# ericehanley/gke-ray-train

Hardware: AMD Instinct MI355X
Metric: tokens/sec (whole node) Llama-2-7B fine-tune at 1/2/4/8 MI355X; samples/sec on Wikitext-2 (higher is better)
Workload: dtype bf16; 1 GPU; model=llama2-7b, global_batch=8, seq_len=1024, parallelism=dp1, micro_batch=8, grad_accum=1, optimizer=fused AdamW fp32 states, activation_checkpointing=False, optimizer_overlap=True, forced_collectives=False, library_gemms=offline-tuned

## Files before the change

gke_ray_train_amd/csrc/bindings/ops.cpp:

```cpp
#include <climits>
#include <torch/extension.h>

#include <algorithm>
#include <cmath>
#include <c10/hip/HIPStream.h>
#include <c10/core/DeviceGuard.h>

#include "grt_kernels.h"
#include "grt_sdma.h"

namespace {

using at::Tensor;
using c10::optional;

hipStream_t cur_stream(const Tensor& t) {
  return c10::hip::getCurrentHIPStream(t.device().index()).stream();
}

grt::DType dtype_of(const Tensor& t) {
  if (t.scalar_type() == at::kBFloat16) return grt::DType::BF16;
  TORCH_CHECK(t.scalar_type() == at::kFloat, "gke_ray_train_amd kernels support bf16/fp32, got ", t.scalar_type());
  return grt::DType::F32;
}
// ... 697 lines not shown
  if (p.drop_thresh == 0) p.drop_thresh = 1;
  p.drop_scale = (float)(1.0 / (1.0 - dropout_p));
}

std::vector<Tensor> attn_fwd(const Tensor& q, const Tensor& k, const Tensor& v, const optional<Tensor>& out,
                             double scale, bool causal, const optional<Tensor>& seqlens_k, double dropout_p,
                             int64_t seed, const optional<Tensor>& cu_seqlens, int64_t max_seqlen,
                             const optional<Tensor>& o_t) {
  c10::OptionalDeviceGuard g(q.device());
  Tensor o = out.has_value() ? *out : at::empty(q.sizes(), q.options());
  auto lse = cu_seqlens.has_value()
                 ? at::empty({cu_seqlens->numel() - 1, q.size(2), max_seqlen}, q.options().dtype(at::kFloat))
                 : at::empty({q.size(0), q.size(2), q.size(1)}, q.options().dtype(at::kFloat));
  auto p = make_params(q, k, v, o, lse, scale, causal, seqlens_k, cu_seqlens, max_seqlen);
  set_dropout(p, dropout_p, seed);
  if (o_t.has_value()) {
    check_contig(*o_t, "o_t");
    TORCH_CHECK(q.scalar_type() == at::kBFloat16 && p.D == 128 && o_t->scalar_type() == at::kBFloat16 &&
                    o_t->dim() == 2 && o_t->size(0) == (int64_t)p.Hq * p.D && o_t->size(1) == q.size(0) * q.size(1),
                "attn_fwd o_t: bf16, head_dim 128, shape [Hq * D, B * S]");
    p.o_t = o_t->data_ptr();
    p.ot_ld = o_t->size(1);
  }
  if (q.scalar_type() == at::kFloat) grt::attn_fwd_f32(p, cur_stream(q));
  else grt::attn_fwd(p, cur_stream(q));
  return {o, lse};
}

std::vector<Tensor> attn_bwd(const Tensor& dout, const Tensor& q, const Tensor& k, const Tensor& v, const Tensor& o,
                             Tensor& lse, const optional<Tensor>& dq_out, const optional<Tensor>& dk_out,
                             const optional<Tensor>& dv_out, double scale, bool causal,
                             const optional<Tensor>& seqlens_k, double dropout_p, int64_t seed,
                             const optional<Tensor>& rope_cos, const optional<Tensor>& rope_sin,
                             const optional<Tensor>& cu_seqlens, int64_t max_seqlen, const optional<Tensor>& dqkv_t) {
  c10::OptionalDeviceGuard g(q.device());
  check_bshd(dout, "dout");
  TORCH_CHECK(dout.sizes() == q.sizes(), "dout shape");
  auto p = make_params(q, k, v, o, lse, scale, causal, seqlens_k, cu_seqlens, max_seqlen);
  set_dropout(p, dropout_p, seed);
  Tensor dq = dq_out.has_value() ? *dq_out : at::empty(q.sizes(), q.options());
  Tensor dk = dk_out.has_value() ? *dk_out : at::empty(k.sizes(), k.options());
  Tensor dv = dv_out.has_value() ? *dv_out : at::empty(v.sizes(), v.options());
  check_bshd(dq, "dq");
  check_bshd(dk, "dk");
  check_bshd(dv, "dv");
  TORCH_CHECK(dq.sizes() == q.sizes() && dk.sizes() == k.sizes() && dv.sizes() == v.sizes(), "grad shapes");
  auto ws = at::empty({grt::attn_bwd_workspace_floats(p.B, p.Hq, p.Sq, p.D)}, q.options().dtype(at::kFloat));
  grt::AttnBwdParams bp{};
  bp.f = p;
  bp.dout = dout.data_ptr(); bp.do_bs = dout.stride(0); bp.do_ss = dout.stride(1); bp.do_hs = dout.stride(2);
  bp.dq = dq.data_ptr(); bp.dq_bs = dq.stride(0); bp.dq_ss = dq.stride(1); bp.dq_hs = dq.stride(2);
  bp.dk = dk.data_ptr(); bp.dk_bs = dk.stride(0); bp.dk_ss = dk.stride(1); bp.dk_hs = dk.stride(2);
  bp.dv = dv.data_ptr(); bp.dv_bs = dv.stride(0); bp.dv_ss = dv.stride(1); bp.dv_hs = dv.stride(2);
  if (cu_seqlens.has_value()) bp.do_bs = bp.dq_bs = bp.dk_bs = bp.dv_bs = 0;
  bp.delta = ws.data_ptr<float>();
  TORCH_CHECK(rope_cos.has_value() == rope_sin.has_value(), "attn_bwd: rope_cos and rope_sin together");
  if (rope_cos.has_value()) {
    check_contig(*rope_cos, "rope_cos");
    check_contig(*rope_sin, "rope_sin");
    TORCH_CHECK(q.scalar_type() == at::kBFloat16 && p.D == 128, "attn_bwd rope epilogue: bf16, head_dim 128");
    TORCH_CHECK(rope_cos->scalar_type() == at::kFloat && rope_sin->sizes() == rope_cos->sizes() &&
                    rope_sin->scalar_type() == at::kFloat && rope_cos->dim() == 2 && rope_cos->size(1) == p.D / 2 &&
                    rope_cos->size(0) >= std::max(p.Sq, p.Sk),
                "attn_bwd: rope tables fp32 [>= max(Sq, Sk), D / 2]");
    bp.rope_cos = rope_cos->data_ptr<float>();
    bp.rope_sin = rope_sin->data_ptr<float>();
  }
  TORCH_CHECK(dout.scalar_type() == q.scalar_type() && dq.scalar_type() == q.scalar_type() &&
                  dk.scalar_type() == q.scalar_type() && dv.scalar_type() == q.scalar_type(), "grad dtype mismatch");
  if (dqkv_t.has_value()) {
    check_contig(*dqkv_t, "dqkv_t");
    TORCH_CHECK(q.scalar_type() == at::kBFloat16 && p.D == 128 && dqkv_t->scalar_type() == at::kBFloat16,
                "attn_bwd dqkv_t: bf16, head_dim 128");
    TORCH_CHECK(p.Sq == p.Sk && dqkv_t->dim() == 2 && dqkv_t->size(0) == (int64_t)(p.Hq + 2 * p.Hkv) * p.D &&
                    dqkv_t->size(1) == q.size(0) * q.size(1),
                "attn_bwd dqkv_t: self-attention, shape [(Hq + 2 Hkv) * D, B * S]");
    bp.dqkv_t = dqkv_t->data_ptr();
    bp.t_ld = dqkv_t->size(1);
    bp.t_row_q = 0;
    bp.t_row_k = p.Hq * p.D;
    bp.t_row_v = (p.Hq + p.Hkv) * p.D;
  }
  if (q.scalar_type() == at::kFloat) grt::attn_bwd_f32(bp, cur_stream(q));
  else grt::attn_bwd(bp, cur_stream(q));
  return {dq, dk, dv};
}

Tensor attn_decode(const Tensor& q, const Tensor& k, const Tensor& v, const optional<Tensor>& seqlens_k, double scale) {
  check_bshd(q, "q");
  check_bshd(k, "k");
  check_bshd(v, "v");
  TORCH_CHECK(q.scalar_type() == at::kBFloat16 && k.scalar_type() == at::kBFloat16 && v.scalar_type() == at::kBFloat16,
              "attn_decode: bf16");
  TORCH_CHECK(q.size(1) == 1, "attn_decode: one query token per sequence");
  TORCH_CHECK(k.sizes() == v.sizes() && k.size(0) == q.size(0), "attn_decode: k/v shapes");
  const int64_t Hq = q.size(2), Hkv = k.size(2);
  TORCH_CHECK(Hq % Hkv == 0, "attn_decode: Hq % Hkv");
  const int64_t G = Hq / Hkv;
  TORCH_CHECK(G == 1 || G == 2 || G == 4 || G == 8, "attn_decode: GQA group must be 1, 2, 4 or 8");
  c10::OptionalDeviceGuard g(q.device());
  grt::AttnDecodeParams p{};
  p.q = q.data_ptr(); p.k = k.data_ptr(); p.v = v.data_ptr();
  auto o = at::empty(q.sizes(), q.options());
  p.o = o.data_ptr();
  p.q_bs = q.stride(0); p.q_hs = q.stride(2);
  p.k_bs = k.stride(0); p.k_ss = k.stride(1); p.k_hs = k.stride(2);
  p.v_bs = v.stride(0); p.v_ss = v.stride(1); p.v_hs = v.stride(2);
  p.o_bs = o.stride(0); p.o_hs = o.stride(2);
  p.B = (int)q.size(0); p.Hq = (int)Hq; p.Hkv = (int)Hkv; p.Sk = (int)k.size(1);
  p.NS = grt::attn_decode_splits(p.B, p.Hkv, p.Sk);
  p.seqlens_k = nullptr;
  if (seqlens_k.has_value()) {
    check_contig(*seqlens_k, "seqlens_k");
    TORCH_CHECK(seqlens_k->scalar_type() == at::kInt && seqlens_k->numel() == q.size(0), "seqlens_k int32 [B]");
    p.seqlens_k = seqlens_k->data_ptr<int32_t>();
  }
  p.scale_log2 = (float)(scale * 1.4426950408889634);
// ... 436 lines not shown
        py::arg("want_xd"), py::arg("h_out") = py::none(), py::arg("hscale") = 1.0);
  m.def("lora_dx", &lora_dx, py::arg("g"), py::arg("at"), py::arg("dx"), py::arg("p"), py::arg("seed"),
        py::arg("offset"), py::arg("accumulate"), py::arg("dx_in") = py::none(), py::arg("gscale") = 1.0);
  m.def("lora_refresh", &lora_refresh, py::arg("bs"), py::arg("offs"), py::arg("w"), py::arg("wt"), py::arg("col0"),
        py::arg("wt_row0") = -1);
  m.def("lora_g", &lora_g, py::arg("a"), py::arg("bt"), py::arg("c"), py::arg("alpha"), py::arg("accumulate"));
  m.def("lora_g_group", &lora_g_group, py::arg("a"), py::arg("bt"), py::arg("c"), py::arg("alpha"),
        py::arg("accumulate"));
  m.def("lora_tred", &lora_tred, py::arg("a"), py::arg("h"), py::arg("out"), py::arg("alpha"), py::arg("accumulate"),
        py::arg("transpose"));
  m.def("lora_tred_group", &lora_tred_group, py::arg("a"), py::arg("h"), py::arg("out"), py::arg("alpha"),
        py::arg("accumulate"));
  m.def("dropout_bwd_seeded", &dropout_bwd_seeded);
  m.def("ce_fwd", &ce_fwd);
  m.def("ce_bwd", &ce_bwd);
  m.def("sumsq_blocks", &sumsq_blocks);
  m.def("lds_fill", [](int64_t pattern, int64_t device) {
    c10::OptionalDeviceGuard g(c10::Device(c10::DeviceType::CUDA, (c10::DeviceIndex)device));
    grt::lds_fill((uint32_t)pattern, c10::hip::getCurrentHIPStream((c10::DeviceIndex)device).stream());
  }, "test support: fill every CU's LDS with a 32-bit pattern (stale-LDS-read detection)");
  m.def("sumsq", &sumsq);
  m.def("clip_finalize", &clip_finalize);
  m.def("adamw", &adamw, py::arg("p"), py::arg("g"), py::arg("m"), py::arg("v"), py::arg("master"),
        py::arg("hyper"), py::arg("gscale"), py::arg("max_blocks") = 0, py::arg("index_offset") = 0);
  m.def("adamw_t", &adamw_t);
  m.def("scale_", &scale_);
  m.def("attn_fwd", &attn_fwd, py::arg("q"), py::arg("k"), py::arg("v"), py::arg("out"), py::arg("scale"),
        py::arg("causal"), py::arg("seqlens_k"), py::arg("dropout_p") = 0.0, py::arg("seed") = 0,
        py::arg("cu_seqlens") = py::none(), py::arg("max_seqlen") = 0, py::arg("o_t") = py::none());
  m.def("attn_bwd", &attn_bwd, py::arg("dout"), py::arg("q"), py::arg("k"), py::arg("v"), py::arg("o"),
        py::arg("lse"), py::arg("dq"), py::arg("dk"), py::arg("dv"), py::arg("scale"), py::arg("causal"),
        py::arg("seqlens_k"), py::arg("dropout_p") = 0.0, py::arg("seed") = 0, py::arg("rope_cos") = py::none(),
        py::arg("rope_sin") = py::none(), py::arg("cu_seqlens") = py::none(), py::arg("max_seqlen") = 0,
        py::arg("dqkv_t") = py::none());
  m.def("attn_set_schedule", &grt::attn_set_schedule,
        "bf16 attention causal-pair / XCD-grouped schedule, bit mask: 1 = forward, 2 = dQ, 4 = dK/dV");
  m.def("attn_get_schedule", &grt::attn_get_schedule);
  m.def("attn_set_dkdv_form", &grt::attn_set_dkdv_form, "dK / dV kernel: 1 = 4-wave, 2 = wave-pair (default)");
  m.def("attn_get_dkdv_form", &grt::attn_get_dkdv_form);
  m.def("attn_set_dma_fast", &grt::attn_set_dma_fast, "1 = hoisted LDS-DMA addressing (default), 0 = clamped per tile");
  m.def("ew_set_fast", &grt::ew_set_fast, "1 = single-pass RoPE (D = 128) / SwiGLU kernels (default), 0 = grid-stride kernels");
  m.def("attn_set_skip_dead", &grt::attn_set_skip_dead,
        "1 = forward / dK-dV waves skip the causal tiles they mask entirely (default), 0 = compute them");
  m.def("nf4_quantize", &nf4_quantize);
  m.def("nf4_dequantize", &nf4_dequantize);
  m.def("nf4_dequantize_t", &nf4_dequantize_t);
  m.def("nf4_dequantize_into", &nf4_dequantize_into);
  m.def("rmsnorm_bwd_dx", &rmsnorm_bwd_dx);
  m.def("swiglu_fwd_t", &swiglu_fwd_t);
  m.def("swiglu_bwd_t", &swiglu_bwd_t);
  m.def("transpose_into", &transpose_into);
  m.def("copy_sdma", &copy_sdma);
  m.def("sdma_d2h", &sdma_d2h, py::arg("dst"), py::arg("src"), py::arg("producer_stream") = 0,
        "pinned host <- device on an SDMA engine, ordered on the source's current stream; producer_stream "
        "(a raw stream handle): the stream whose work so far wrote src");
  m.def("sdma_stats", &sdma_stats, "copies / bytes / worker busy seconds / first error of the SDMA copier");
  m.def("sdma_clear_error", [](int64_t device) { grt::sdma_clear_error((int)device); });
  m.def("gemv", &gemv, py::arg("x"), py::arg("w"), py::arg("swiglu") = false);
  m.def("gemv_fused", &gemv_fused, py::arg("x"), py::arg("w"), py::arg("sumsq"), py::arg("slot"),
        py::arg("swiglu") = false, py::arg("g") = py::none(), py::arg("res") = py::none(), py::arg("eps") = 1e-5,
        py::arg("cos") = py::none(), py::arg("sin") = py::none(), py::arg("pos") = py::none(),
        py::arg("kc") = py::none(), py::arg("vc") = py::none(), py::arg("hq") = 0, py::arg("hkv") = 0);
  m.def("attn_decode", &attn_decode);
  m.def("embedding_fwd", &embedding_fwd);
  m.def("embedding_bwd", &embedding_bwd);
  m.def("gemm_wgrad", &gemm_wgrad, py::arg("x"), py::arg("y"), py::arg("out"), py::arg("accumulate"),
        py::arg("mode") = 0);
// ... 18 lines not shown
```

gke_ray_train_amd/csrc/kernels/attention.hip:

```cpp
#include <limits.h>
#include <stdlib.h>

#include <type_traits>
#include <utility>

#include "grt_common.h"
#include "grt_kernels.h"

namespace grt {
namespace {

typedef __attribute__((address_space(3))) bf16x4 lds_bf16x4;

constexpr int D = 128;
constexpr int kChunks = D / 8;

__device__ __forceinline__ f32x16 mfma32(bf16x8 a, bf16x8 b, f32x16 c) {
  return __builtin_amdgcn_mfma_f32_32x32x16_bf16(a, b, c, 0, 0, 0);
}

__device__ __forceinline__ int img_off(int row, int ch) {
  return row * 256 + 16 * (ch ^ (((row & 3) << 2) | ((row >> 2) & 3)));
}
__device__ __forceinline__ bf16x8 lds_row_read(const char* base, int row, int ch) {
// ... 6 lines not shown
  return __builtin_amdgcn_ds_read_tr16_b64_v4bf16((lds_bf16x4*)a);
}

__device__ __forceinline__ bf16x8 cat(bf16x4 a, bf16x4 b) {
  return __builtin_shufflevector(a, b, 0, 1, 2, 3, 4, 5, 6, 7);
}
__device__ __forceinline__ bf16x8 pack8(const f32x16& x, int base) {
  bf16x8 r;
#pragma unroll
  for (int j = 0; j < 8; ++j) r[j] = static_cast<bf16>(x[base + j]);
  return r;
}
__device__ __forceinline__ int acc_row(int r, int h) { return (r & 3) + 8 * (r >> 2) + 4 * h; }

__device__ __forceinline__ uint32_t fmix32(uint32_t h) {
  h ^= h >> 16; h *= 0x85ebca6bu; h ^= h >> 13; h *= 0xc2b2ae35u; h ^= h >> 16;
  return h;
}
__device__ __forceinline__ uint32_t attn_dropout_hash(uint32_t seed, uint32_t bh, uint32_t q, uint32_t k) {
  uint32_t h = seed ^ (bh * 0x9E3779B1u);
  h = fmix32(h ^ (q * 0x85EBCA77u));
  return fmix32(h ^ (k * 0xC2B2AE3Du));
}
__device__ __forceinline__ float drop_factor(const AttnParams& p, uint32_t bh, int q, int k) {
  return attn_dropout_hash(p.drop_seed, bh, (uint32_t)q, (uint32_t)k) >= p.drop_thresh ? p.drop_scale : 0.f;
}

constexpr float kLog2e = 1.4426950408889634f;
constexpr float kLn2 = 0.6931471805599453f;

__device__ __forceinline__ float halves_max(float x) {
  const auto r = __builtin_amdgcn_permlane32_swap(__float_as_uint(x), __float_as_uint(x), false, false);
  return fmaxf(__uint_as_float(r[0]), __uint_as_float(r[1]));
}

constexpr float kDeferLog2 = 8.f;

__device__ __forceinline__ void lds_dma16(const void* gptr, uint32_t lds_byte_addr) {
  asm volatile("s_mov_b32 m0, %1\n\ts_nop 0\n\tglobal_load_lds_dwordx4 %0, off"
               :: "v"(gptr), "s"(lds_byte_addr) : "memory", "m0");
}
__device__ __forceinline__ uint32_t lds_u32(const void* p) {
  return (uint32_t)(uintptr_t)(const __attribute__((address_space(3))) char*)(p);
}
__device__ __forceinline__ int img_swz(int row) { return ((row & 3) << 2) | ((row >> 2) & 3); }

template <class F, int... I>
__device__ __forceinline__ void static_for(F&& f, std::integer_sequence<int, I...>) {
  (f(std::integral_constant<int, I>{}), ...);
}
__device__ __forceinline__ void wait_tiles4(int tiles) {
  if (tiles >= 4) asm volatile("s_waitcnt vmcnt(16)" ::: "memory");
  else if (tiles == 3) asm volatile("s_waitcnt vmcnt(12)" ::: "memory");
  else if (tiles == 2) asm volatile("s_waitcnt vmcnt(8)" ::: "memory");
  else if (tiles == 1) asm volatile("s_waitcnt vmcnt(4)" ::: "memory");
  else asm volatile("s_waitcnt vmcnt(0)" ::: "memory");
}

constexpr int F3M = 128, F3N = 32, F3NT = 256, F3NSLOT = 4;
constexpr int F3IMG = F3N * D * 2;
constexpr int F3SLOT = 2 * F3IMG;

struct QJobs {
  int bh;
  int blk0, blk1;
};
// ... 212 lines not shown
        a.v[j] = static_cast<bf16>(o[db][8 * gp + j] * inv);
        c2.v[j] = static_cast<bf16>(o[db][8 * gp + 4 + j] * inv);
      }
      const auto r0 = __builtin_amdgcn_permlane32_swap(a.u[0], c2.u[0], false, false);
      const auto r1 = __builtin_amdgcn_permlane32_swap(a.u[1], c2.u[1], false, false);
      if (myq < Sq) {
        *reinterpret_cast<uint4*>(O + db * 32 + 16 * gp + 8 * h) = make_uint4(r0[0], r1[0], r0[1], r1[1]);
        if (p.o_t != nullptr) {
          bf16* ot = static_cast<bf16*>(p.o_t) + (int64_t)(hq * D) * p.ot_ld + (p.cu_seqlens ? 0 : (int64_t)b * p.Sq) +
                     tok0 + myq;
          const int d0 = db * 32 + 8 * (2 * gp) + 4 * h, d1 = db * 32 + 8 * (2 * gp + 1) + 4 * h;
#pragma unroll
          for (int j = 0; j < 4; ++j) {
            ot[(int64_t)(d0 + j) * p.ot_ld] = a.v[j];
            ot[(int64_t)(d1 + j) * p.ot_ld] = c2.v[j];
          }
        }
      }
    }
  if (myq < Sq) {
    if (h == 0 && p.lse)
      p.lse[((int64_t)b * p.Hq + hq) * p.Sq + myq] = lt > 0.f ? (m + __log2f(lt)) * kLn2 : INFINITY;
  }
  };
  run_block(jobs.blk0);
  if (jobs.blk1 >= 0) {
    asm volatile("s_waitcnt lgkmcnt(0)" ::: "memory");
    __builtin_amdgcn_s_barrier();
    run_block(jobs.blk1);
  }
}

__host__ __device__ inline int sq_pad(int Sq) { return (Sq + 31) / 32 * 32; }

__global__ __launch_bounds__(256) void attn_bwd_pre_kernel(const AttnBwdParams p) {
  const int l16 = threadIdx.x & 15;
  const int Sqp = sq_pad(p.f.Sq);
  const int64_t row = (int64_t)blockIdx.x * 16 + (threadIdx.x >> 4);
  const int64_t nrows = (int64_t)p.f.B * p.f.Hq * Sqp;
  if (row >= nrows) return;
  const int q = (int)(row % Sqp);
  const int64_t bh = row / Sqp;
  float acc = 0.f;
  const int hq = (int)(bh % p.f.Hq), b = (int)(bh / p.f.Hq);
  int Sq = p.f.Sq;
  int64_t tok0 = 0;
  if (p.f.cu_seqlens) {
    tok0 = p.f.cu_seqlens[b];
    Sq = p.f.cu_seqlens[b + 1] - (int)tok0;
  }
  if (q < Sq) {
    const bf16* O = (const bf16*)p.f.o + (int64_t)b * p.f.o_bs + (int64_t)hq * p.f.o_hs + (tok0 + q) * p.f.o_ss;
    const bf16* dO = (const bf16*)p.dout + (int64_t)b * p.do_bs + (int64_t)hq * p.do_hs + (tok0 + q) * p.do_ss;
    float a[8], g[8];
    load16(O + l16 * 8, a);
    load16(dO + l16 * 8, g);
#pragma unroll
    for (int k = 0; k < 8; ++k) acc += a[k] * g[k];
  }
#pragma unroll
  for (int o = 8; o >= 1; o >>= 1) acc += __shfl_xor(acc, o, 16);
  if (l16 == 0) {
    float* lse2 = p.delta + nrows;
    p.delta[row] = acc;
    lse2[row] = q < Sq ? p.f.lse[bh * p.f.Sq + q] * kLog2e : INFINITY;
  }
}


struct TCopy {
  bf16* p;
  int64_t ld;
};
__device__ __forceinline__ void st_t(const TCopy& tc, int d, const bf16x4& v) {
  if (tc.p != nullptr) {
#pragma unroll
    for (int j = 0; j < 4; ++j) tc.p[(int64_t)(d + j) * tc.ld] = v[j];
  }
}
__device__ __forceinline__ TCopy tcopy(const AttnBwdParams& P, int row0, int head, int64_t tok) {
  if (P.dqkv_t == nullptr) return TCopy{nullptr, 0};
  return TCopy{static_cast<bf16*>(P.dqkv_t) + (int64_t)(row0 + head * D) * P.t_ld + tok, P.t_ld};
}

__device__ __forceinline__ void store_unrotated(const f32x16 (&acc)[4], float scale, const float* __restrict__ cr,
                                                const float* __restrict__ sr, bf16* dst, int h,
                                                const TCopy& tc = TCopy{nullptr, 0}) {
#pragma unroll
  for (int db = 0; db < 2; ++db)
#pragma unroll
    for (int gg = 0; gg < 4; ++gg) {
      const int d = db * 32 + 8 * gg + 4 * h;
      const f32x4 c = *reinterpret_cast<const f32x4*>(cr + d);
      const f32x4 sn = *reinterpret_cast<const f32x4*>(sr + d);
      bf16x4 lo, hi;
#pragma unroll
      for (int j = 0; j < 4; ++j) {
        const float x1 = acc[db][4 * gg + j] * scale, x2 = acc[db + 2][4 * gg + j] * scale;
        lo[j] = static_cast<bf16>(x1 * c[j] + x2 * sn[j]);
        hi[j] = static_cast<bf16>(x2 * c[j] - x1 * sn[j]);
      }
// ... 536 lines not shown
  auto run_role = [&](auto role_c) __attribute__((always_inline)) {
    run_block(jobs.blk0, role_c);
    if (jobs.blk1 >= 0) {
      asm volatile("s_waitcnt lgkmcnt(0)" ::: "memory");
      __builtin_amdgcn_s_barrier();
      run_block(jobs.blk1, role_c);
    }
  };
  if (swave) run_role(std::true_type{});
  else run_role(std::false_type{});
}

constexpr int Q2M = 128, Q2N = 32, Q2NT = 256, Q2NSLOT = 4;
constexpr int Q2IMG = Q2N * D * 2;
constexpr int Q2SLOT = 2 * Q2IMG;

template <bool DROP>
__global__ __launch_bounds__(Q2NT, 2) void attn_bwd_dq_kernel(const AttnBwdParams P) {
  const AttnParams& p = P.f;
  __shared__ __attribute__((aligned(16))) char smem[Q2NSLOT * Q2SLOT];
  const int tid = threadIdx.x, lane = tid & 63, h = lane >> 5, l32 = lane & 31;
  const int w = __builtin_amdgcn_readfirstlane(tid >> 6);
  const int g = lane >> 4, l16 = lane & 15;
  const int nqb = (p.Sq + Q2M - 1) / Q2M;
  const int BH = p.B * p.Hq;
  const QJobs jobs = q_jobs(p.sched, nqb, BH);
  const int bh = jobs.bh;
  const int b = bh / p.Hq, hq = bh % p.Hq;
  const int hkv = hq / (p.Hq / p.Hkv);
  GRT_DEVICE_CHECK(b < p.B && hkv < p.Hkv && jobs.blk0 >= 0 && jobs.blk0 < nqb);
  auto run_block = [&](const int qblk) {
  int Sq = p.Sq, Sk = p.Sk;
  int64_t tok0 = 0;
  if (p.cu_seqlens) {
    tok0 = p.cu_seqlens[b];
    Sq = Sk = p.cu_seqlens[b + 1] - (int)tok0;
    if (qblk * Q2M >= Sq) return;
  }
  const int sk = p.seqlens_k ? min(Sk, p.seqlens_k[b]) : Sk;
  const int off = Sk - Sq;
  const int q0 = qblk * Q2M, qw0 = q0 + w * 32;
  const int myq = qw0 + l32;
  const bool qok = myq < Sq;
  const int Sqp = sq_pad(p.Sq);

  const bf16* Q = (const bf16*)p.q + (int64_t)b * p.q_bs + tok0 * p.q_ss + (int64_t)hq * p.q_hs;
  const bf16* dO = (const bf16*)P.dout + (int64_t)b * P.do_bs + tok0 * P.do_ss + (int64_t)hq * P.do_hs;
  const bf16* K = (const bf16*)p.k + (int64_t)b * p.k_bs + tok0 * p.k_ss + (int64_t)hkv * p.k_hs;
  const bf16* Vg = (const bf16*)p.v + (int64_t)b * p.v_bs + tok0 * p.v_ss + (int64_t)hkv * p.v_hs;

  bf16x8 qf[D / 16], of[D / 16];
#pragma unroll
  for (int ks = 0; ks < D / 16; ++ks) {
    if (qok) {
      qf[ks] = *reinterpret_cast<const bf16x8*>(Q + (int64_t)myq * p.q_ss + ks * 16 + 8 * h);
      of[ks] = *reinterpret_cast<const bf16x8*>(dO + (int64_t)myq * P.do_ss + ks * 16 + 8 * h);
    } else {
      qf[ks] = bf16x8{};
      of[ks] = bf16x8{};
    }
  }
  const int64_t ri = (int64_t)bh * Sqp + min(myq, Sqp - 1);
  const float lse2 = P.delta[(int64_t)BH * Sqp + ri];
  const float dlt = P.delta[ri];
  const float c = p.scale * kLog2e;
  const int klim = p.causal ? min(sk - 1, myq + off) : sk - 1;
  const int kmask = p.causal ? min(sk, qw0 + off + 1) : sk;
  const int klast = p.skip_dead && p.causal && !DROP ? min(sk - 1, qw0 + 31 + off) : INT_MAX;

  int kend = sk;
  if (p.causal) kend = min(kend, q0 + Q2M + off);
  const int nt = kend > 0 ? (kend + Q2N - 1) / Q2N : 0;

  const uint32_t smem0 = lds_u32(smem);
  const int row0 = 8 * w + g, row1 = row0 + 4;
  const int ch0 = l16 ^ img_swz(row0), ch1 = l16 ^ img_swz(row1);
  auto dma_tile = [&](int t, uint32_t slot_off) {
    const int64_t k0r = min(t * Q2N + row0, Sk - 1), k1r = min(t * Q2N + row1, Sk - 1);
    const uint32_t dst = __builtin_amdgcn_readfirstlane(smem0 + slot_off + (uint32_t)(8 * w * 256));
    lds_dma16(K + k0r * p.k_ss + ch0 * 8, dst);
    lds_dma16(Vg + k0r * p.v_ss + ch0 * 8, dst + Q2IMG);
    lds_dma16(K + k1r * p.k_ss + ch1 * 8, dst + 1024);
    lds_dma16(Vg + k1r * p.v_ss + ch1 * 8, dst + Q2IMG + 1024);
  };
  auto wait_dma = [&](int pending_tiles) {
    if (pending_tiles >= 2) asm volatile("s_waitcnt vmcnt(8)" ::: "memory");
    else if (pending_tiles == 1) asm volatile("s_waitcnt vmcnt(4)" ::: "memory");
    else asm volatile("s_waitcnt vmcnt(0)" ::: "memory");
  };
  auto sdp = [&](int t, auto slot_c, f32x16& s, f32x16& dp) {
    constexpr int SL = decltype(slot_c)::value;
    const char* ki = smem + SL * Q2SLOT;
    const int kb = t * Q2N;
    s = f32x16{};
    if (kb + Q2N > kmask) {
#pragma unroll
      for (int r = 0; r < 16; ++r) s[r] = kb + acc_row(r, h) <= klim ? 0.f : -INFINITY;
// ... 24 lines not shown
  for (int i = 0; i < 4; ++i) dq[i] = f32x16{};

  using I0 = std::integral_constant<int, 0>;
  auto step = [&](int t, auto slot_c, f32x16& s_c, f32x16& dp_c, f32x16& s_n, f32x16& dp_n) {
    constexpr int SL = decltype(slot_c)::value;
    asm volatile("s_waitcnt lgkmcnt(0)" ::: "memory");
    if (t + 1 < nt) wait_dma(min(nt, t + Q2NSLOT - 1) - (t + 2));
    __builtin_amdgcn_s_barrier();
    if (t + Q2NSLOT - 1 < nt) dma_tile(t + Q2NSLOT - 1, (uint32_t)(((SL + Q2NSLOT - 1) % Q2NSLOT) * Q2SLOT));
    if (t * Q2N > klast) return;

    sdp(t + 1, std::integral_constant<int, (SL + 1) % Q2NSLOT>{}, s_n, dp_n);

#pragma unroll
    for (int r = 0; r < 16; ++r) {
      const float pv = fast_exp2(fmaf(s_c[r], c, -lse2));
      const float z = DROP ? drop_factor(p, (uint32_t)bh, myq, t * Q2N + acc_row(r, h)) : 1.f;
      s_c[r] = pv * (dp_c[r] * z - dlt);
    }
    const char* ki = smem + SL * Q2SLOT;
#pragma unroll
    for (int stp = 0; stp < 2; ++stp) {
      const bf16x8 sb = pack8(s_c, 8 * stp);
      const int kk = 16 * stp + 4 * h;
#pragma unroll
      for (int db = 0; db < 4; ++db) {
        const int c0 = db * 32 + (g & 1) * 16;
        const bf16x8 a = cat(lds_tr_read(ki, kk, c0, l16), lds_tr_read(ki, kk + 8, c0, l16));
        dq[db] = mfma32(a, sb, dq[db]);
      }
    }
  };

  if (nt > 0) {
    const int pre = min(nt, Q2NSLOT - 1);
    for (int t = 0; t < pre; ++t) dma_tile(t, (uint32_t)(t * Q2SLOT));
    wait_dma(pre - 1);
    __builtin_amdgcn_s_barrier();
    f32x16 sA, dpA, sB, dpB;
    sdp(0, I0{}, sA, dpA);
    int t = 0;
    for (; t + Q2NSLOT <= nt; t += Q2NSLOT) {
      step(t, I0{}, sA, dpA, sB, dpB);
      step(t + 1, std::integral_constant<int, 1>{}, sB, dpB, sA, dpA);
      step(t + 2, std::integral_constant<int, 2>{}, sA, dpA, sB, dpB);
      step(t + 3, std::integral_constant<int, 3>{}, sB, dpB, sA, dpA);
    }
    if (t < nt) step(t, I0{}, sA, dpA, sB, dpB);
    if (t + 1 < nt) step(t + 1, std::integral_constant<int, 1>{}, sB, dpB, sA, dpA);
    if (t + 2 < nt) step(t + 2, std::integral_constant<int, 2>{}, sA, dpA, sB, dpB);
  }
  asm volatile("s_waitcnt vmcnt(0)" ::: "memory");

  if (qok) {
    bf16* dQ = (bf16*)P.dq + (int64_t)b * P.dq_bs + (int64_t)hq * P.dq_hs + (tok0 + myq) * P.dq_ss;
    const TCopy tq = tcopy(P, P.t_row_q, hq, (p.cu_seqlens ? 0 : (int64_t)b * p.Sq) + tok0 + myq);
    if (P.rope_cos) {
      store_unrotated(dq, p.scale, P.rope_cos + (int64_t)myq * (D / 2), P.rope_sin + (int64_t)myq * (D / 2), dQ, h, tq);
    } else {
#pragma unroll
      for (int db = 0; db < 4; ++db)
#pragma unroll
        for (int gg = 0; gg < 4; ++gg) {
          bf16x4 v;
#pragma unroll
          for (int j = 0; j < 4; ++j) v[j] = static_cast<bf16>(dq[db][4 * gg + j] * p.scale);
          *reinterpret_cast<bf16x4*>(dQ + db * 32 + 8 * gg + 4 * h) = v;
          st_t(tq, db * 32 + 8 * gg + 4 * h, v);
        }
// ... 41 lines not shown
static int pair_if_fills(int want, int nblk, int groups, int per_cu) {
  return want && (int64_t)groups * ((nblk + 1) / 2) >= (int64_t)cu_count() * per_cu ? 1 : 0;
}

void attn_set_schedule(int s) { g_sched = s; }
void attn_set_dkdv_form(int f) { g_dkdv = f == 1 ? 1 : 2; }
int attn_get_dkdv_form() { return g_dkdv; }
void attn_set_dma_fast(int on) { g_dma_fast = on ? 1 : 0; }
void attn_set_skip_dead(int on) { g_skip_dead = on ? 1 : 0; }
int attn_get_schedule() { return g_sched; }

static int sched_for(const AttnParams& p, int bit) { return p.cu_seqlens ? 0 : (g_sched >> bit) & 1; }

void attn_fwd(const AttnParams& p0, hipStream_t s) {
  AttnParams p = p0;
  p.dma_fast = dma_fast_for(p, 0);
  p.skip_dead = skip_dead_now();
  const int nqb = (p.Sq + F3M - 1) / F3M;
  p.sched = pair_if_fills(sched_for(p, 0), nqb, p.B * p.Hq, 2);
  const dim3 grid(q_grid(p.sched, nqb, p.B * p.Hq));
  if (p.drop_thresh) hipLaunchKernelGGL((attn_fwd_kernel<true, F3NSLOT>), grid, dim3(F3NT), 0, s, p);
  else hipLaunchKernelGGL((attn_fwd_kernel<false, F3NSLOT>), grid, dim3(F3NT), 0, s, p);
}

int64_t attn_bwd_workspace_floats(int B, int Hq, int Sq, int Dh) {
  (void)Dh;
  return 2 * (int64_t)B * Hq * sq_pad(Sq);
}

void attn_bwd(const AttnBwdParams& p0, hipStream_t s) {
  AttnBwdParams p = p0;
  p.f.dma_fast = dma_fast_for(p.f, p.do_ss);
  p.f.skip_dead = skip_dead_now();
  const int64_t rows = (int64_t)p.f.B * p.f.Hq * sq_pad(p.f.Sq);
  hipLaunchKernelGGL(attn_bwd_pre_kernel, dim3((unsigned)((rows + 15) / 16)), dim3(256), 0, s, p);
  const int nkb = (p.f.Sk + K2N - 1) / K2N;
  const int nqb = (p.f.Sq + Q2M - 1) / Q2M;
  AttnBwdParams pk = p, pq = p;
  pk.f.sched = pair_if_fills(sched_for(p.f, 2), nkb, p.f.B * p.f.Hkv, 1);
  pq.f.sched = pair_if_fills(sched_for(p.f, 1), nqb, p.f.B * p.f.Hq, 2);
  const dim3 g1(q_grid(pk.f.sched, nkb, p.f.B * p.f.Hkv)), g2(q_grid(pq.f.sched, nqb, p.f.B * p.f.Hq));
  static_assert(K3N == K2N, "both dK / dV forms take 128-key blocks (same grid)");
  if (p.f.drop_thresh) {
    hipLaunchKernelGGL(attn_bwd_dkdv_kernel<true>, g1, dim3(K2NT), 0, s, pk);
    hipLaunchKernelGGL(attn_bwd_dq_kernel<true>, g2, dim3(Q2NT), 0, s, pq);
  } else {
    if (g_dkdv == 2) hipLaunchKernelGGL(attn_bwd_dkdv2_kernel, g1, dim3(K3NT), 0, s, pk);
    else hipLaunchKernelGGL(attn_bwd_dkdv_kernel<false>, g1, dim3(K2NT), 0, s, pk);
    hipLaunchKernelGGL(attn_bwd_dq_kernel<false>, g2, dim3(Q2NT), 0, s, pq);
  }
}

}
```

gke_ray_train_amd/csrc/kernels/norm.hip:

```cpp
#include <stdlib.h>

#include "grt_common.h"
#include "grt_kernels.h"

namespace grt {
namespace {

constexpr int kNT = 256;
constexpr int kRowsPerBlock = kNT / kWave;
constexpr int kBwdMaxBlocks = 512;

template <typename T, int MAXC, bool RMS, bool RES, bool FULL>
__global__ __launch_bounds__(kNT) void norm_fwd_kernel(const T* __restrict__ x,
                                                       const T* __restrict__ res,
                                                       const T* __restrict__ w,
                                                       const T* __restrict__ b, T* __restrict__ y,
                                                       T* __restrict__ h_out, float* __restrict__ mean_out,
                                                       float* __restrict__ rstd_out, int64_t rows,
                                                       int d, float eps, int64_t ldy) {
  constexpr int V = Vec16<T>::N;
  typedef typename Vec16<T>::type VT;
  const int lane = threadIdx.x & 63;
  const int64_t row = (int64_t)blockIdx.x * kRowsPerBlock + (threadIdx.x >> 6);
  if (row >= rows) return;
// ... 121 lines not shown
        if (!RMS) dbp[c][i] += dv;
      }
    }
    sgx = wave_sum(sgx);
    if (!RMS) sg = wave_sum(sg);
    if (lane == 0) { red[wid] = sgx; red[kRowsPerBlock + wid] = sg; }
    __syncthreads();
    float tsgx = 0.f, tsg = 0.f;
#pragma unroll
    for (int i = 0; i < kRowsPerBlock; ++i) { tsgx += red[i]; tsg += red[kRowsPerBlock + i]; }
    __syncthreads();
    tsgx /= d;
    tsg = RMS ? 0.f : tsg / d;
#pragma unroll
    for (int c = 0; c < MAXC; ++c) {
      const int ch = tid + c * kNT;
      if (ch < nchunk) {
        float o[V];
#pragma unroll
        for (int i = 0; i < V; ++i) o[i] = (RES ? to_f(rc[c][i]) : 0.f) + r * (g[c][i] - tsg - xh[c][i] * tsgx);
        store16(dx + row * d + ch * V, o);
      }
    }
  }
  if (ws == nullptr) return;
  float* wsb = ws + (int64_t)blockIdx.x * 2 * d;
#pragma unroll
  for (int c = 0; c < MAXC; ++c) {
    const int ch = tid + c * kNT;
    if (ch < nchunk) {
#pragma unroll
      for (int i = 0; i < V; ++i) {
        wsb[ch * V + i] = dwp[c][i];
        wsb[d + ch * V + i] = dbp[c][i];
      }
    }
  }
}

constexpr int kColsumCols = 16;
constexpr int kColsumGroups = kNT / kColsumCols;
template <typename GO, bool ACC>
__global__ __launch_bounds__(kNT) void colsum_kernel(const float* __restrict__ ws, int nb, int d, int ncols,
                                                     GO* __restrict__ dw, GO* __restrict__ db) {
  __shared__ float red[kColsumGroups][kColsumCols];
  const int c = threadIdx.x % kColsumCols, rg = threadIdx.x / kColsumCols;
  const int j = blockIdx.x * kColsumCols + c;
  float a0 = 0.f, a1 = 0.f, a2 = 0.f, a3 = 0.f;
  if (j < ncols) {
    const int64_t ld = 2 * (int64_t)d;
    constexpr int G = kColsumGroups;
    int b = rg;
    for (; b + 3 * G < nb; b += 4 * G) {
      a0 += ws[(int64_t)b * ld + j];
      a1 += ws[(int64_t)(b + G) * ld + j];
      a2 += ws[(int64_t)(b + 2 * G) * ld + j];
      a3 += ws[(int64_t)(b + 3 * G) * ld + j];
    }
    for (; b < nb; b += G) a0 += ws[(int64_t)b * ld + j];
  }
  red[rg][c] = (a0 + a1) + (a2 + a3);
  __syncthreads();
  if (rg == 0 && j < ncols) {
    float s = 0.f;
#pragma unroll
    for (int g = 0; g < kColsumGroups; ++g) s += red[g][c];
    GO* out = j < d ? dw : db;
// ... 122 lines not shown
```

Measured before the change: 27600 tokens/s.

## Fuse attention backward preprocessing into dQ kernel and reorder launches

Removes the separate attention-backward preprocessing kernel. The dQ kernel now computes delta (rowsum of O·dO) and the scaled LSE itself and writes them to the workspace, and it is launched before the dK/dV kernel, which reads those stats. A caller can also pass a preallocated workspace to skip the per-call allocation. The RMSNorm backward no longer writes the unused bias-gradient half of its workspace. In exchange the dQ kernel loads O as well, which adds register pressure, and the dK/dV kernel now has to wait for the whole dQ kernel rather than a short preprocessing pass.

```diff
diff --git a/gke_ray_train_amd/csrc/bindings/ops.cpp b/gke_ray_train_amd/csrc/bindings/ops.cpp
--- a/gke_ray_train_amd/csrc/bindings/ops.cpp
+++ b/gke_ray_train_amd/csrc/bindings/ops.cpp
@@ -753,7 +753,8 @@
                              const optional<Tensor>& dv_out, double scale, bool causal,
                              const optional<Tensor>& seqlens_k, double dropout_p, int64_t seed,
                              const optional<Tensor>& rope_cos, const optional<Tensor>& rope_sin,
-                             const optional<Tensor>& cu_seqlens, int64_t max_seqlen, const optional<Tensor>& dqkv_t) {
+                             const optional<Tensor>& cu_seqlens, int64_t max_seqlen, const optional<Tensor>& dqkv_t,
+                             const optional<Tensor>& workspace) {
   c10::OptionalDeviceGuard g(q.device());
   check_bshd(dout, "dout");
   TORCH_CHECK(dout.sizes() == q.sizes(), "dout shape");
@@ -766,7 +767,13 @@
   check_bshd(dk, "dk");
   check_bshd(dv, "dv");
   TORCH_CHECK(dq.sizes() == q.sizes() && dk.sizes() == k.sizes() && dv.sizes() == v.sizes(), "grad shapes");
-  auto ws = at::empty({grt::attn_bwd_workspace_floats(p.B, p.Hq, p.Sq, p.D)}, q.options().dtype(at::kFloat));
+  const int64_t ws_floats = grt::attn_bwd_workspace_floats(p.B, p.Hq, p.Sq, p.D);
+  if (workspace.has_value()) {
+    check_contig(*workspace, "workspace");
+    TORCH_CHECK(workspace->scalar_type() == at::kFloat && workspace->device() == q.device() &&
+                    workspace->numel() >= ws_floats, "attn_bwd workspace: fp32, at least ", ws_floats, " elements");
+  }
+  Tensor ws = workspace.has_value() ? *workspace : at::empty({ws_floats}, q.options().dtype(at::kFloat));
   grt::AttnBwdParams bp{};
   bp.f = p;
   bp.dout = dout.data_ptr(); bp.do_bs = dout.stride(0); bp.do_ss = dout.stride(1); bp.do_hs = dout.stride(2);
@@ -1306,7 +1313,7 @@
         py::arg("lse"), py::arg("dq"), py::arg("dk"), py::arg("dv"), py::arg("scale"), py::arg("causal"),
         py::arg("seqlens_k"), py::arg("dropout_p") = 0.0, py::arg("seed") = 0, py::arg("rope_cos") = py::none(),
         py::arg("rope_sin") = py::none(), py::arg("cu_seqlens") = py::none(), py::arg("max_seqlen") = 0,
-        py::arg("dqkv_t") = py::none());
+        py::arg("dqkv_t") = py::none(), py::arg("workspace") = py::none());
   m.def("attn_set_schedule", &grt::attn_set_schedule,
         "bf16 attention causal-pair / XCD-grouped schedule, bit mask: 1 = forward, 2 = dQ, 4 = dK/dV");
   m.def("attn_get_schedule", &grt::attn_get_schedule);
diff --git a/gke_ray_train_amd/csrc/kernels/attention.hip b/gke_ray_train_amd/csrc/kernels/attention.hip
--- a/gke_ray_train_amd/csrc/kernels/attention.hip
+++ b/gke_ray_train_amd/csrc/kernels/attention.hip
@@ -340,40 +340,6 @@
 }
 
 __host__ __device__ inline int sq_pad(int Sq) { return (Sq + 31) / 32 * 32; }
-
-__global__ __launch_bounds__(256) void attn_bwd_pre_kernel(const AttnBwdParams p) {
-  const int l16 = threadIdx.x & 15;
-  const int Sqp = sq_pad(p.f.Sq);
-  const int64_t row = (int64_t)blockIdx.x * 16 + (threadIdx.x >> 4);
-  const int64_t nrows = (int64_t)p.f.B * p.f.Hq * Sqp;
-  if (row >= nrows) return;
-  const int q = (int)(row % Sqp);
-  const int64_t bh = row / Sqp;
-  float acc = 0.f;
-  const int hq = (int)(bh % p.f.Hq), b = (int)(bh / p.f.Hq);
-  int Sq = p.f.Sq;
-  int64_t tok0 = 0;
-  if (p.f.cu_seqlens) {
-    tok0 = p.f.cu_seqlens[b];
-    Sq = p.f.cu_seqlens[b + 1] - (int)tok0;
-  }
-  if (q < Sq) {
-    const bf16* O = (const bf16*)p.f.o + (int64_t)b * p.f.o_bs + (int64_t)hq * p.f.o_hs + (tok0 + q) * p.f.o_ss;
-    const bf16* dO = (const bf16*)p.dout + (int64_t)b * p.do_bs + (int64_t)hq * p.do_hs + (tok0 + q) * p.do_ss;
-    float a[8], g[8];
-    load16(O + l16 * 8, a);
-    load16(dO + l16 * 8, g);
-#pragma unroll
-    for (int k = 0; k < 8; ++k) acc += a[k] * g[k];
-  }
-#pragma unroll
-  for (int o = 8; o >= 1; o >>= 1) acc += __shfl_xor(acc, o, 16);
-  if (l16 == 0) {
-    float* lse2 = p.delta + nrows;
-    p.delta[row] = acc;
-    lse2[row] = q < Sq ? p.f.lse[bh * p.f.Sq + q] * kLog2e : INFINITY;
-  }
-}
 
 
 struct TCopy {
@@ -977,37 +943,60 @@
   auto run_block = [&](const int qblk) {
   int Sq = p.Sq, Sk = p.Sk;
   int64_t tok0 = 0;
+  const int q0 = qblk * Q2M, qw0 = q0 + w * 32;
+  const int myq = qw0 + l32;
+  const int Sqp = sq_pad(p.Sq);
+  auto put_stats = [&](float dl, float ls) {
+    if (h == 0 && myq < Sqp) {
+      float* st = P.delta + (int64_t)bh * Sqp + myq;
+      st[0] = dl;
+      st[(int64_t)BH * Sqp] = ls;
+    }
+  };
   if (p.cu_seqlens) {
     tok0 = p.cu_seqlens[b];
     Sq = Sk = p.cu_seqlens[b + 1] - (int)tok0;
-    if (qblk * Q2M >= Sq) return;
+    if (qblk * Q2M >= Sq) {
+      put_stats(0.f, INFINITY);
+      return;
+    }
   }
   const int sk = p.seqlens_k ? min(Sk, p.seqlens_k[b]) : Sk;
   const int off = Sk - Sq;
-  const int q0 = qblk * Q2M, qw0 = q0 + w * 32;
-  const int myq = qw0 + l32;
   const bool qok = myq < Sq;
-  const int Sqp = sq_pad(p.Sq);
 
   const bf16* Q = (const bf16*)p.q + (int64_t)b * p.q_bs + tok0 * p.q_ss + (int64_t)hq * p.q_hs;
   const bf16* dO = (const bf16*)P.dout + (int64_t)b * P.do_bs + tok0 * P.do_ss + (int64_t)hq * P.do_hs;
   const bf16* K = (const bf16*)p.k + (int64_t)b * p.k_bs + tok0 * p.k_ss + (int64_t)hkv * p.k_hs;
   const bf16* Vg = (const bf16*)p.v + (int64_t)b * p.v_bs + tok0 * p.v_ss + (int64_t)hkv * p.v_hs;
 
-  bf16x8 qf[D / 16], of[D / 16];
-#pragma unroll
-  for (int ks = 0; ks < D / 16; ++ks) {
-    if (qok) {
+  bf16x8 qf[D / 16], of[D / 16], og[D / 16];
+  float lse2 = INFINITY;
+  if (qok) {
+    const bf16* Orow = (const bf16*)p.o + (int64_t)b * p.o_bs + (int64_t)hq * p.o_hs + (tok0 + myq) * p.o_ss;
+#pragma unroll
+    for (int ks = 0; ks < D / 16; ++ks) {
       qf[ks] = *reinterpret_cast<const bf16x8*>(Q + (int64_t)myq * p.q_ss + ks * 16 + 8 * h);
       of[ks] = *reinterpret_cast<const bf16x8*>(dO + (int64_t)myq * P.do_ss + ks * 16 + 8 * h);
-    } else {
-      qf[ks] = bf16x8{};
-      of[ks] = bf16x8{};
-    }
-  }
-  const int64_t ri = (int64_t)bh * Sqp + min(myq, Sqp - 1);
-  const float lse2 = P.delta[(int64_t)BH * Sqp + ri];
-  const float dlt = P.delta[ri];
+      og[ks] = *reinterpret_cast<const bf16x8*>(Orow + ks * 16 + 8 * h);
+    }
+    lse2 = p.lse[(int64_t)bh * p.Sq + myq] * kLog2e;
+  } else {
+#pragma unroll
+    for (int ks = 0; ks < D / 16; ++ks) { qf[ks] = bf16x8{}; of[ks] = bf16x8{}; og[ks] = bf16x8{}; }
+  }
+  static_assert(D == 128, "the reduction tree below is written for 16 chunks");
+  float cs[D / 16];
+#pragma unroll
+  for (int ks = 0; ks < D / 16; ++ks) {
+    float a = 0.f;
+#pragma unroll
+    for (int k = 0; k < 8; ++k) a += to_f(og[ks][k]) * to_f(of[ks][k]);
+    cs[ks] = a;
+  }
+  float dlt = ((cs[0] + cs[4]) + (cs[2] + cs[6])) + ((cs[1] + cs[5]) + (cs[3] + cs[7]));
+  dlt += __shfl_xor(dlt, 32, 64);
+  put_stats(dlt, lse2);
   const float c = p.scale * kLog2e;
   const int klim = p.causal ? min(sk - 1, myq + off) : sk - 1;
   const int kmask = p.causal ? min(sk, qw0 + off + 1) : sk;
@@ -1208,8 +1197,6 @@
   AttnBwdParams p = p0;
   p.f.dma_fast = dma_fast_for(p.f, p.do_ss);
   p.f.skip_dead = skip_dead_now();
-  const int64_t rows = (int64_t)p.f.B * p.f.Hq * sq_pad(p.f.Sq);
-  hipLaunchKernelGGL(attn_bwd_pre_kernel, dim3((unsigned)((rows + 15) / 16)), dim3(256), 0, s, p);
   const int nkb = (p.f.Sk + K2N - 1) / K2N;
   const int nqb = (p.f.Sq + Q2M - 1) / Q2M;
   AttnBwdParams pk = p, pq = p;
@@ -1218,13 +1205,13 @@
   const dim3 g1(q_grid(pk.f.sched, nkb, p.f.B * p.f.Hkv)), g2(q_grid(pq.f.sched, nqb, p.f.B * p.f.Hq));
   static_assert(K3N == K2N, "both dK / dV forms take 128-key blocks (same grid)");
   if (p.f.drop_thresh) {
+    hipLaunchKernelGGL(attn_bwd_dq_kernel<true>, g2, dim3(Q2NT), 0, s, pq);
     hipLaunchKernelGGL(attn_bwd_dkdv_kernel<true>, g1, dim3(K2NT), 0, s, pk);
-    hipLaunchKernelGGL(attn_bwd_dq_kernel<true>, g2, dim3(Q2NT), 0, s, pq);
   } else {
+    hipLaunchKernelGGL(attn_bwd_dq_kernel<false>, g2, dim3(Q2NT), 0, s, pq);
     if (g_dkdv == 2) hipLaunchKernelGGL(attn_bwd_dkdv2_kernel, g1, dim3(K3NT), 0, s, pk);
     else hipLaunchKernelGGL(attn_bwd_dkdv_kernel<false>, g1, dim3(K2NT), 0, s, pk);
-    hipLaunchKernelGGL(attn_bwd_dq_kernel<false>, g2, dim3(Q2NT), 0, s, pq);
-  }
-}
-
-}
+  }
+}
+
+}
diff --git a/gke_ray_train_amd/csrc/kernels/norm.hip b/gke_ray_train_amd/csrc/kernels/norm.hip
--- a/gke_ray_train_amd/csrc/kernels/norm.hip
+++ b/gke_ray_train_amd/csrc/kernels/norm.hip
@@ -177,7 +177,7 @@
 #pragma unroll
       for (int i = 0; i < V; ++i) {
         wsb[ch * V + i] = dwp[c][i];
-        wsb[d + ch * V + i] = dbp[c][i];
+        if (!RMS) wsb[d + ch * V + i] = dbp[c][i];
       }
     }
   }
```

Result: no change. 27670 tokens/s (median of 6 runs) (+0.3%).

## Fold attention backward delta/lse preprocessing into the dQ kernel

Applied to the files above, without the earlier changes.

Removes the separate attention-backward preprocessing kernel. The dQ kernel now loads O, computes delta = rowsum(dO*O) and the scaled lse itself, overlapping that work with its initial K/V tile prefetch, and writes both values to the workspace. The dQ kernel is launched before dK/dV so the dK/dV kernel can read those stats. This saves one launch and one extra pass over O and dO, at the cost of more registers and loads in the dQ kernel, and it serialises dK/dV behind dQ. An optional return_stats flag exposes the workspace.

```diff
diff --git a/gke_ray_train_amd/csrc/bindings/ops.cpp b/gke_ray_train_amd/csrc/bindings/ops.cpp
--- a/gke_ray_train_amd/csrc/bindings/ops.cpp
+++ b/gke_ray_train_amd/csrc/bindings/ops.cpp
@@ -753,7 +753,8 @@
                              const optional<Tensor>& dv_out, double scale, bool causal,
                              const optional<Tensor>& seqlens_k, double dropout_p, int64_t seed,
                              const optional<Tensor>& rope_cos, const optional<Tensor>& rope_sin,
-                             const optional<Tensor>& cu_seqlens, int64_t max_seqlen, const optional<Tensor>& dqkv_t) {
+                             const optional<Tensor>& cu_seqlens, int64_t max_seqlen, const optional<Tensor>& dqkv_t,
+                             bool return_stats) {
   c10::OptionalDeviceGuard g(q.device());
   check_bshd(dout, "dout");
   TORCH_CHECK(dout.sizes() == q.sizes(), "dout shape");
@@ -804,6 +805,7 @@
   }
   if (q.scalar_type() == at::kFloat) grt::attn_bwd_f32(bp, cur_stream(q));
   else grt::attn_bwd(bp, cur_stream(q));
+  if (return_stats) return {dq, dk, dv, ws.view({2, (int64_t)p.B * p.Hq, -1})};
   return {dq, dk, dv};
 }
 
@@ -1306,7 +1308,7 @@
         py::arg("lse"), py::arg("dq"), py::arg("dk"), py::arg("dv"), py::arg("scale"), py::arg("causal"),
         py::arg("seqlens_k"), py::arg("dropout_p") = 0.0, py::arg("seed") = 0, py::arg("rope_cos") = py::none(),
         py::arg("rope_sin") = py::none(), py::arg("cu_seqlens") = py::none(), py::arg("max_seqlen") = 0,
-        py::arg("dqkv_t") = py::none());
+        py::arg("dqkv_t") = py::none(), py::arg("return_stats") = false);
   m.def("attn_set_schedule", &grt::attn_set_schedule,
         "bf16 attention causal-pair / XCD-grouped schedule, bit mask: 1 = forward, 2 = dQ, 4 = dK/dV");
   m.def("attn_get_schedule", &grt::attn_get_schedule);
diff --git a/gke_ray_train_amd/csrc/kernels/attention.hip b/gke_ray_train_amd/csrc/kernels/attention.hip
--- a/gke_ray_train_amd/csrc/kernels/attention.hip
+++ b/gke_ray_train_amd/csrc/kernels/attention.hip
@@ -62,6 +62,10 @@
 __device__ __forceinline__ float halves_max(float x) {
   const auto r = __builtin_amdgcn_permlane32_swap(__float_as_uint(x), __float_as_uint(x), false, false);
   return fmaxf(__uint_as_float(r[0]), __uint_as_float(r[1]));
+}
+__device__ __forceinline__ float halves_sum(float x) {
+  const auto r = __builtin_amdgcn_permlane32_swap(__float_as_uint(x), __float_as_uint(x), false, false);
+  return __uint_as_float(r[0]) + __uint_as_float(r[1]);
 }
 
 constexpr float kDeferLog2 = 8.f;
@@ -340,41 +344,6 @@
 }
 
 __host__ __device__ inline int sq_pad(int Sq) { return (Sq + 31) / 32 * 32; }
-
-__global__ __launch_bounds__(256) void attn_bwd_pre_kernel(const AttnBwdParams p) {
-  const int l16 = threadIdx.x & 15;
-  const int Sqp = sq_pad(p.f.Sq);
-  const int64_t row = (int64_t)blockIdx.x * 16 + (threadIdx.x >> 4);
-  const int64_t nrows = (int64_t)p.f.B * p.f.Hq * Sqp;
-  if (row >= nrows) return;
-  const int q = (int)(row % Sqp);
-  const int64_t bh = row / Sqp;
-  float acc = 0.f;
-  const int hq = (int)(bh % p.f.Hq), b = (int)(bh / p.f.Hq);
-  int Sq = p.f.Sq;
-  int64_t tok0 = 0;
-  if (p.f.cu_seqlens) {
-    tok0 = p.f.cu_seqlens[b];
-    Sq = p.f.cu_seqlens[b + 1] - (int)tok0;
-  }
-  if (q < Sq) {
-    const bf16* O = (const bf16*)p.f.o + (int64_t)b * p.f.o_bs + (int64_t)hq * p.f.o_hs + (tok0 + q) * p.f.o_ss;
-    const bf16* dO = (const bf16*)p.dout + (int64_t)b * p.do_bs + (int64_t)hq * p.do_hs + (tok0 + q) * p.do_ss;
-    float a[8], g[8];
-    load16(O + l16 * 8, a);
-    load16(dO + l16 * 8, g);
-#pragma unroll
-    for (int k = 0; k < 8; ++k) acc += a[k] * g[k];
-  }
-#pragma unroll
-  for (int o = 8; o >= 1; o >>= 1) acc += __shfl_xor(acc, o, 16);
-  if (l16 == 0) {
-    float* lse2 = p.delta + nrows;
-    p.delta[row] = acc;
-    lse2[row] = q < Sq ? p.f.lse[bh * p.f.Sq + q] * kLog2e : INFINITY;
-  }
-}
-
 
 struct TCopy {
   bf16* p;
@@ -977,37 +946,51 @@
   auto run_block = [&](const int qblk) {
   int Sq = p.Sq, Sk = p.Sk;
   int64_t tok0 = 0;
+  const int q0 = qblk * Q2M, qw0 = q0 + w * 32;
+  const int myq = qw0 + l32;
+  const int Sqp = sq_pad(p.Sq);
+  float* const st_delta = P.delta + (int64_t)bh * Sqp + myq;
+  float* const st_lse2 = st_delta + (int64_t)BH * Sqp;
+  const bool st_w = h == 0 && myq < Sqp;
   if (p.cu_seqlens) {
     tok0 = p.cu_seqlens[b];
     Sq = Sk = p.cu_seqlens[b + 1] - (int)tok0;
-    if (qblk * Q2M >= Sq) return;
+    if (qblk * Q2M >= Sq) {
+      if (st_w) {
+        *st_delta = 0.f;
+        *st_lse2 = INFINITY;
+      }
+      return;
+    }
   }
   const int sk = p.seqlens_k ? min(Sk, p.seqlens_k[b]) : Sk;
   const int off = Sk - Sq;
-  const int q0 = qblk * Q2M, qw0 = q0 + w * 32;
-  const int myq = qw0 + l32;
   const bool qok = myq < Sq;
-  const int Sqp = sq_pad(p.Sq);
 
   const bf16* Q = (const bf16*)p.q + (int64_t)b * p.q_bs + tok0 * p.q_ss + (int64_t)hq * p.q_hs;
   const bf16* dO = (const bf16*)P.dout + (int64_t)b * P.do_bs + tok0 * P.do_ss + (int64_t)hq * P.do_hs;
   const bf16* K = (const bf16*)p.k + (int64_t)b * p.k_bs + tok0 * p.k_ss + (int64_t)hkv * p.k_hs;
   const bf16* Vg = (const bf16*)p.v + (int64_t)b * p.v_bs + tok0 * p.v_ss + (int64_t)hkv * p.v_hs;
 
-  bf16x8 qf[D / 16], of[D / 16];
-#pragma unroll
-  for (int ks = 0; ks < D / 16; ++ks) {
-    if (qok) {
+  bf16x8 qf[D / 16], of[D / 16], oc[D / 16];
+  float lse2 = INFINITY, dlt = 0.f;
+  if (qok) {
+    const bf16* Og = (const bf16*)p.o + (int64_t)b * p.o_bs + tok0 * p.o_ss + (int64_t)hq * p.o_hs;
+    lse2 = p.lse[(int64_t)bh * p.Sq + myq];
+#pragma unroll
+    for (int ks = 0; ks < D / 16; ++ks) {
       qf[ks] = *reinterpret_cast<const bf16x8*>(Q + (int64_t)myq * p.q_ss + ks * 16 + 8 * h);
       of[ks] = *reinterpret_cast<const bf16x8*>(dO + (int64_t)myq * P.do_ss + ks * 16 + 8 * h);
-    } else {
+      oc[ks] = *reinterpret_cast<const bf16x8*>(Og + (int64_t)myq * p.o_ss + ks * 16 + 8 * h);
+    }
+  } else {
+#pragma unroll
+    for (int ks = 0; ks < D / 16; ++ks) {
       qf[ks] = bf16x8{};
       of[ks] = bf16x8{};
-    }
-  }
-  const int64_t ri = (int64_t)bh * Sqp + min(myq, Sqp - 1);
-  const float lse2 = P.delta[(int64_t)BH * Sqp + ri];
-  const float dlt = P.delta[ri];
+      oc[ks] = bf16x8{};
+    }
+  }
   const float c = p.scale * kLog2e;
   const int klim = p.causal ? min(sk - 1, myq + off) : sk - 1;
   const int kmask = p.causal ? min(sk, qw0 + off + 1) : sk;
@@ -1098,9 +1081,21 @@
     }
   };
 
+  const int pre = min(nt, Q2NSLOT - 1);
+  for (int t = 0; t < pre; ++t) dma_tile(t, (uint32_t)(t * Q2SLOT));
+#pragma unroll
+  for (int ks = 0; ks < D / 16; ++ks)
+#pragma unroll
+    for (int j = 0; j < 8; ++j) dlt = fmaf(static_cast<float>(of[ks][j]), static_cast<float>(oc[ks][j]), dlt);
+  dlt = halves_sum(dlt);
+  asm volatile("" : "+v"(lse2));
+  lse2 *= kLog2e;
+  if (st_w) {
+    *st_delta = dlt;
+    *st_lse2 = lse2;
+  }
+
   if (nt > 0) {
-    const int pre = min(nt, Q2NSLOT - 1);
-    for (int t = 0; t < pre; ++t) dma_tile(t, (uint32_t)(t * Q2SLOT));
     wait_dma(pre - 1);
     __builtin_amdgcn_s_barrier();
     f32x16 sA, dpA, sB, dpB;
@@ -1208,8 +1203,6 @@
   AttnBwdParams p = p0;
   p.f.dma_fast = dma_fast_for(p.f, p.do_ss);
   p.f.skip_dead = skip_dead_now();
-  const int64_t rows = (int64_t)p.f.B * p.f.Hq * sq_pad(p.f.Sq);
-  hipLaunchKernelGGL(attn_bwd_pre_kernel, dim3((unsigned)((rows + 15) / 16)), dim3(256), 0, s, p);
   const int nkb = (p.f.Sk + K2N - 1) / K2N;
   const int nqb = (p.f.Sq + Q2M - 1) / Q2M;
   AttnBwdParams pk = p, pq = p;
@@ -1218,13 +1211,13 @@
   const dim3 g1(q_grid(pk.f.sched, nkb, p.f.B * p.f.Hkv)), g2(q_grid(pq.f.sched, nqb, p.f.B * p.f.Hq));
   static_assert(K3N == K2N, "both dK / dV forms take 128-key blocks (same grid)");
   if (p.f.drop_thresh) {
+    hipLaunchKernelGGL(attn_bwd_dq_kernel<true>, g2, dim3(Q2NT), 0, s, pq);
     hipLaunchKernelGGL(attn_bwd_dkdv_kernel<true>, g1, dim3(K2NT), 0, s, pk);
-    hipLaunchKernelGGL(attn_bwd_dq_kernel<true>, g2, dim3(Q2NT), 0, s, pq);
   } else {
+    hipLaunchKernelGGL(attn_bwd_dq_kernel<false>, g2, dim3(Q2NT), 0, s, pq);
     if (g_dkdv == 2) hipLaunchKernelGGL(attn_bwd_dkdv2_kernel, g1, dim3(K3NT), 0, s, pk);
     else hipLaunchKernelGGL(attn_bwd_dkdv_kernel<false>, g1, dim3(K2NT), 0, s, pk);
-    hipLaunchKernelGGL(attn_bwd_dq_kernel<false>, g2, dim3(Q2NT), 0, s, pq);
-  }
-}
-
-}
+  }
+}
+
+}
```

After: 28200 tokens/s before, 28280 tokens/s after (median of 2 runs). Within noise of the previous version (+0.3%).
